# IIT-PAVIS/DiffAssemble

Measured on AMD Instinct MI355X. Metric: denoising steps/sec (900-piece dense graph, T=100), higher is better.
Workload: dtype bf16

## Files before the change

diffassemble_amd/csrc/da_basic.hip:

```cpp
#include "da_common.h"
#include "da_internal.h"

namespace da {

template <typename T>
__global__ __launch_bounds__(256) void k_set_feats(int n, int F, int D, const float *__restrict__ feats,
                                                   T *__restrict__ comb_in) {
    size_t total = (size_t)n * F;
    for (size_t idx = (size_t)blockIdx.x * blockDim.x + threadIdx.x; idx < total;
         idx += (size_t)gridDim.x * blockDim.x) {
        size_t r = idx / F;
        int c = (int)(idx - r * F);
        stf(comb_in + r * D + c, feats[idx]);
    }
}

template <typename T>
__global__ __launch_bounds__(256) void k_set_virtual_rows(int rows, int V, int D, const T *__restrict__ emb,
                                                          T *__restrict__ dst) {
    size_t total = (size_t)rows * D;
    for (size_t idx = (size_t)blockIdx.x * blockDim.x + threadIdx.x; idx < total;
         idx += (size_t)gridDim.x * blockDim.x) {
        size_t r = idx / D;
        int c = (int)(idx - r * D);
        dst[idx] = emb[(size_t)(r % V) * D + c];
    }
}

template <typename T>
__global__ __launch_bounds__(256) void k_embed_pos_time(int n, int NPW, int c_in, int F, int D, const float *__restrict__ x,
                                                        const int64_t *__restrict__ t, int64_t t_scalar, int steps,
                                                        const float *__restrict__ time_emb,
                                                        const float *__restrict__ w0, const float *__restrict__ b0,
                                                        const float *__restrict__ w1, const float *__restrict__ b1,
                                                        T *__restrict__ comb_in, int embed_blocks, VirtScatter vs) {
    __shared__ float hid[4][16];
    if ((int)blockIdx.x >= embed_blocks) {
        const int HC = vs.H * vs.C;
        const size_t total = (size_t)vs.rows * 4 * HC, stride = (size_t)(gridDim.x - embed_blocks) * blockDim.x;
        for (size_t idx = (size_t)(blockIdx.x - embed_blocks) * blockDim.x + threadIdx.x; idx < total; idx += stride) {
            const size_t r = idx / (4 * (size_t)HC);
            const int col = (int)(idx - r * 4 * HC), which = col / HC, f = col - which * HC;
            const T v = ((const T *)vs.src)[(size_t)(r % vs.V) * 4 * HC + col];
            const size_t node = (size_t)vs.n_real + r;
            if (which == 3) { ((T *)vs.S)[node * HC + f] = v; continue; }
            const int h = f / vs.C, c = f - h * vs.C;
            T *dstb = (T *)(which == 0 ? vs.Q : (which == 1 ? vs.K : vs.Vt));
            dstb[((size_t)h * (size_t)vs.n_pad + (size_t)vs.row_map[node]) * vs.C + c] = v;
        }
        return;
    }
    const int lane = threadIdx.x & 63, wv = threadIdx.x >> 6;
    const int r0 = (blockIdx.x * 4 + wv) * NPW;
    if (r0 >= n) return;
    float w0r[8], w1r[16];
    float b0r = 0.f, b1r = 0.f;
    if (lane < 16) {
        b0r = b0[lane];
#pragma unroll
        for (int k = 0; k < 8; ++k) w0r[k] = k < c_in ? w0[lane * c_in + k] : 0.f;
    }
    if (lane < 32) {
        b1r = b1[lane];
#pragma unroll
        for (int k = 0; k < 16; ++k) w1r[k] = w1[lane * 16 + k];
    }
    for (int i = 0; i < NPW; ++i) {
        const int r = r0 + i;
        if (r >= n) break;
        if (lane < 16) {
            float a = b0r;
#pragma unroll
            for (int k = 0; k < 8; ++k) a += k < c_in ? w0r[k] * x[(size_t)r * c_in + k] : 0.f;
            hid[wv][lane] = gelu_erf(a);
        }
        __builtin_amdgcn_wave_barrier();
        asm volatile("s_waitcnt lgkmcnt(0)" ::: "memory");
        T *dst = comb_in + (size_t)r * D + F;
        if (lane < 32) {
            float a = b1r;
#pragma unroll
            for (int k = 0; k < 16; ++k) a += w1r[k] * hid[wv][k];
            stf(dst + lane, a);
        } else {
            int64_t ti = t ? t[r] : t_scalar;
            ti = ti < 0 ? 0 : (ti >= steps ? steps - 1 : ti);
            stf(dst + lane, time_emb[ti * 32 + (lane - 32)]);
        }
        __builtin_amdgcn_wave_barrier();
    }
}

template <typename T>
__global__ __launch_bounds__(256) void k_gemm_simple(int M, int K, int Nout, const T *__restrict__ A, int lda,
                                                     const T *__restrict__ W, const float *__restrict__ bias,
                                                     int act, const T *__restrict__ res, T *__restrict__ out,
                                                     int ldo) {
    __shared__ float As[16][68];
    __shared__ float Ws[16][68];
    const int tx = threadIdx.x & 15, ty = threadIdx.x >> 4;
    const int row0 = blockIdx.y * 64, col0 = blockIdx.x * 64;
    const int lr = threadIdx.x >> 2, lk = (threadIdx.x & 3) * 4;
    float acc[4][4];
#pragma unroll
    for (int i = 0; i < 4; ++i)
#pragma unroll
        for (int j = 0; j < 4; ++j) acc[i][j] = 0.f;
    const int ar = row0 + lr, wr = col0 + lr;
    for (int k0 = 0; k0 < K; k0 += 16) {
#pragma unroll
        for (int i = 0; i < 4; ++i) {
            const int k = k0 + lk + i;
            As[lk + i][lr] = (ar < M && k < K) ? ldf(A + (size_t)ar * lda + k) : 0.f;
            Ws[lk + i][lr] = (wr < Nout && k < K) ? ldf(W + (size_t)wr * K + k) : 0.f;
        }
        __syncthreads();
#pragma unroll
        for (int kk = 0; kk < 16; ++kk) {
            float a[4], b[4];
#pragma unroll
            for (int i = 0; i < 4; ++i) { a[i] = As[kk][ty * 4 + i]; b[i] = Ws[kk][tx * 4 + i]; }
#pragma unroll
            for (int i = 0; i < 4; ++i)
#pragma unroll
                for (int j = 0; j < 4; ++j) acc[i][j] = fmaf(a[i], b[j], acc[i][j]);
        }
        __syncthreads();
    }
#pragma unroll
    for (int i = 0; i < 4; ++i) {
        const int r = row0 + ty * 4 + i;
        if (r >= M) continue;
#pragma unroll
        for (int j = 0; j < 4; ++j) {
            const int c = col0 + tx * 4 + j;
            if (c >= Nout) continue;
            float v = acc[i][j] + (bias ? bias[c] : 0.f);
            v = apply_act(v, act);
            if (res) v += ldf(res + (size_t)r * ldo + c);
            stf(out + (size_t)r * ldo + c, v);
        }
    }
}

template <typename T>
__global__ __launch_bounds__(256) void k_head2d(int n, int c_out, const T *__restrict__ hh,
                                                const float *__restrict__ w2, const float *__restrict__ b2,
                                                float *__restrict__ out) {
    const int idx = blockIdx.x * blockDim.x + threadIdx.x;
    if (idx >= n * c_out) return;
    const int r = idx / c_out, c = idx - r * c_out;
    float a = b2[c];
#pragma unroll
    for (int k = 0; k < 32; ++k) a += w2[c * 32 + k] * ldf(hh + (size_t)r * 32 + k);
    out[idx] = a;
}

__global__ __launch_bounds__(256) void k_ddim2d(DeviceSchedule s, int mean_type, int n, int c,
                                                const float *__restrict__ x, const float *__restrict__ mo,
                                                const int64_t *__restrict__ t, int64_t t_scalar, int ratio,
                                                int prev_all_nonneg, float eta, const float *__restrict__ noise,
                                                float *__restrict__ x_prev) {
    const int idx = blockIdx.x * blockDim.x + threadIdx.x;
    if (idx >= n * c) return;
    const int r = idx / c;
    const int64_t ti = t ? t[r] : t_scalar;
    x_prev[idx] = ddim2d_value(s, mean_type, ti, ratio, prev_all_nonneg, eta, x[idx], mo[idx], (eta > 0.f && noise) ? noise[idx] : 0.f);
}

__global__ __launch_bounds__(256) void k_ddpm2d(DeviceSchedule s, int n, int c, const float *__restrict__ x,
                                                const float *__restrict__ mo, const int64_t *__restrict__ t,
                                                int64_t t_scalar, const float *__restrict__ noise,
                                                float *__restrict__ x_prev) {
    const int idx = blockIdx.x * blockDim.x + threadIdx.x;
    if (idx >= n * c) return;
    const int r = idx / c;
    int64_t ti = t ? t[r] : t_scalar;
    ti = ti < 0 ? 0 : (ti >= s.steps ? s.steps - 1 : ti);
    float mean = s.sqrt_recip_alphas[ti] * (x[idx] - s.betas[ti] * mo[idx] / s.sqrt_one_minus_alphas_cumprod[ti]);
    if (noise) mean += sqrtf(s.posterior_variance[ti]) * noise[idx];
    x_prev[idx] = mean;
}

template <typename T>
__global__ __launch_bounds__(256) void k_convert(size_t n, const float *__restrict__ src, T *__restrict__ dst) {
    for (size_t i = (size_t)blockIdx.x * blockDim.x + threadIdx.x; i < n; i += (size_t)gridDim.x * blockDim.x)
        stf(dst + i, src[i]);
}

static inline int grid_for(size_t total, int block = 256, int cap = 4096) {
    size_t g = (total + block - 1) / block;
    return (int)(g < 1 ? 1 : (g > (size_t)cap ? cap : g));
}

template <typename T>
static int launch_set_feats_t(int n, int F, int D, const float *feats, void *comb_in, hipStream_t st) {
    if (n <= 0) return 0;
    k_set_feats<T><<<grid_for((size_t)n * F), 256, 0, st>>>(n, F, D, feats, (T *)comb_in);
    DA_LAUNCH_CHECK();
    return 0;
}
int launch_set_feats(int prec, int n, int F, int D, const float *feats, void *comb_in, hipStream_t st) {
    return prec == DA_PREC_BF16 ? launch_set_feats_t<bf16_t>(n, F, D, feats, comb_in, st)
                                : launch_set_feats_t<float>(n, F, D, feats, comb_in, st);
}

int launch_set_virtual_rows(int prec, int rows, int V, int D, const void *emb, void *dst, hipStream_t st) {
    if (rows <= 0) return 0;
    if (prec == DA_PREC_BF16)
        k_set_virtual_rows<bf16_t><<<grid_for((size_t)rows * D), 256, 0, st>>>(rows, V, D, (const bf16_t *)emb, (bf16_t *)dst);
    else
        k_set_virtual_rows<float><<<grid_for((size_t)rows * D), 256, 0, st>>>(rows, V, D, (const float *)emb, (float *)dst);
    DA_LAUNCH_CHECK();
    return 0;
}

int launch_embed_pos_time(int prec, int n, int c_in, int F, int D, const float *x, const int64_t *t, int64_t t_scalar,
                          int steps, const float *time_emb, const float *w0, const float *b0, const float *w1,
                          const float *b1, void *comb_in, hipStream_t st, const VirtScatter *vsp) {
    if (n <= 0) return 0;
    if (c_in > 8) { set_error("launch_embed_pos_time: c_in %d > 8", c_in); return 2; }
    VirtScatter vs;
    if (vsp && vsp->rows > 0) vs = *vsp;
    const size_t vtotal = (size_t)vs.rows * 4 * vs.H * vs.C;
    const int vblocks = vs.rows > 0 ? (int)((vtotal + 255) / 256 > 1024 ? 1024 : (vtotal + 255) / 256) : 0;
    const int npw_env = DA_XENV("DA_EMBED_NPW", 0);
    const int npw = npw_env > 0 ? npw_env : (n >= 8192 ? 8 : 1), grid = (n + 4 * npw - 1) / (4 * npw);
    if (prec == DA_PREC_BF16)
        k_embed_pos_time<bf16_t><<<grid + vblocks, 256, 0, st>>>(n, npw, c_in, F, D, x, t, t_scalar, steps, time_emb, w0, b0, w1, b1, (bf16_t *)comb_in, grid, vs);
    else
        k_embed_pos_time<float><<<grid + vblocks, 256, 0, st>>>(n, npw, c_in, F, D, x, t, t_scalar, steps, time_emb, w0, b0, w1, b1, (float *)comb_in, grid, vs);
    DA_LAUNCH_CHECK();
    return 0;
}

int launch_gemm_simple(int prec, int M, int K, int Nout, const void *A, int lda, const void *W, const float *bias,
                       int act, const void *res, void *out, int ldo, hipStream_t st) {
    if (M <= 0 || Nout <= 0) return 0;
    dim3 grid((Nout + 63) / 64, (M + 63) / 64);
    if (prec == DA_PREC_BF16)
        k_gemm_simple<bf16_t><<<grid, 256, 0, st>>>(M, K, Nout, (const bf16_t *)A, lda, (const bf16_t *)W, bias, act, (const bf16_t *)res, (bf16_t *)out, ldo);
    else
        k_gemm_simple<float><<<grid, 256, 0, st>>>(M, K, Nout, (const float *)A, lda, (const float *)W, bias, act, (const float *)res, (float *)out, ldo);
    DA_LAUNCH_CHECK();
    return 0;
}

int launch_head2d(int prec, int n, int c_out, const void *hh, const float *w2, const float *b2, float *out, hipStream_t st) {
    if (n <= 0) return 0;
    const int grid = (n * c_out + 255) / 256;
    if (prec == DA_PREC_BF16)
        k_head2d<bf16_t><<<grid, 256, 0, st>>>(n, c_out, (const bf16_t *)hh, w2, b2, out);
    else
        k_head2d<float><<<grid, 256, 0, st>>>(n, c_out, (const float *)hh, w2, b2, out);
    DA_LAUNCH_CHECK();
    return 0;
}

int launch_ddim2d(const DeviceSchedule &s, int mean_type, int n, int c, const float *x, const float *mo,
                  const int64_t *t, int64_t t_scalar, int ratio, int prev_all_nonneg, float eta, const float *noise,
                  float *x_prev, hipStream_t st) {
    if (n <= 0) return 0;
    k_ddim2d<<<(n * c + 255) / 256, 256, 0, st>>>(s, mean_type, n, c, x, mo, t, t_scalar, ratio, prev_all_nonneg, eta, noise, x_prev);
    DA_LAUNCH_CHECK();
    return 0;
}

int launch_ddpm2d(const DeviceSchedule &s, int n, int c, const float *x, const float *mo, const int64_t *t,
                  int64_t t_scalar, const float *noise, float *x_prev, hipStream_t st) {
    if (n <= 0) return 0;
    k_ddpm2d<<<(n * c + 255) / 256, 256, 0, st>>>(s, n, c, x, mo, t, t_scalar, noise, x_prev);
    DA_LAUNCH_CHECK();
    return 0;
}

int launch_convert(int prec, size_t n, const float *src, void *dst, hipStream_t st) {
    if (n == 0) return 0;
    if (prec == DA_PREC_BF16)
        k_convert<bf16_t><<<grid_for(n), 256, 0, st>>>(n, src, (bf16_t *)dst);
    else
        k_convert<float><<<grid_for(n), 256, 0, st>>>(n, src, (float *)dst);
    DA_LAUNCH_CHECK();
    return 0;
}


__global__ __launch_bounds__(256) void k_mm_nn_f32(int M, int N, int K, const float *__restrict__ A, int lda,
                                                   const float *__restrict__ B, int ldb, const float *__restrict__ bias,
                                                   float *__restrict__ Cm, int ldc) {
    const int idx = blockIdx.x * blockDim.x + threadIdx.x;
    if (idx >= M * N) return;
    const int m = idx / N, n = idx - m * N;
    float acc = 0.f;
    for (int k = 0; k < K; ++k) acc = fmaf(A[(size_t)m * lda + k], B[(size_t)k * ldb + n], acc);
    Cm[(size_t)m * ldc + n] = acc + (bias ? bias[m] : 0.f);
}

int launch_mm_nn_f32(int M, int N, int K, const float *A, int lda, const float *B, int ldb, const float *bias, float *Cm,
                     int ldc, hipStream_t st) {
    k_mm_nn_f32<<<(M * N + 255) / 256, 256, 0, st>>>(M, N, K, A, lda, B, ldb, bias, Cm, ldc);
    DA_LAUNCH_CHECK();
    return 0;
}

__device__ __forceinline__ void ld4f(const float *p, float (&v)[4]) {
    const float4 f = *(const float4 *)p;
    v[0] = f.x; v[1] = f.y; v[2] = f.z; v[3] = f.w;
}
__device__ __forceinline__ void ld4f(const bf16_t *p, float (&v)[4]) {
    const uint2 u = *(const uint2 *)p;
    v[0] = bf2f((bf16_t)(u.x & 0xffff)); v[1] = bf2f((bf16_t)(u.x >> 16));
    v[2] = bf2f((bf16_t)(u.y & 0xffff)); v[3] = bf2f((bf16_t)(u.y >> 16));
}
template <typename T>
__global__ __launch_bounds__(256) void k_head_fold(int n, int H, int c_out, const T *__restrict__ pz, const T *__restrict__ pre,
                                                   const float *__restrict__ w2, const float *__restrict__ b2,
                                                   float *__restrict__ out, DdimFuse df) {
    __shared__ float f[32][33];
    const int q = threadIdx.x & 7, lr = threadIdx.x >> 3;
    const int r = blockIdx.x * 32 + lr;
    if (r < n) {
        float a[4], v[4];
        ld4f(pre + (size_t)r * 32 + 4 * q, a);
        for (int h = 0; h < H; ++h) {
            ld4f(pz + ((size_t)h * n + r) * 32 + 4 * q, v);
#pragma unroll
            for (int e = 0; e < 4; ++e) a[e] += v[e];
        }
#pragma unroll
        for (int e = 0; e < 4; ++e) f[lr][4 * q + e] = gelu_erf(a[e]);
    }
    __syncthreads();
    const int lr2 = threadIdx.x / c_out, j = threadIdx.x - lr2 * c_out;
    const int r2 = blockIdx.x * 32 + lr2;
    if (lr2 < 32 && r2 < n) {
        float a = b2[j];
#pragma unroll
        for (int k = 0; k < 32; ++k) a = fmaf(w2[j * 32 + k], f[lr2][k], a);
        out[(size_t)r2 * c_out + j] = a;
        if (df.x_prev)
            df.x_prev[(size_t)r2 * c_out + j] = ddim2d_value(df.s, df.mean_type, df.t, df.ratio, df.prev_all_nonneg, 0.f,
                                                             df.x[(size_t)r2 * c_out + j], a, 0.f);
    }
}

typedef __attribute__((ext_vector_type(8))) __bf16 tl_bf16x8;
typedef __attribute__((ext_vector_type(16))) float tl_f32x16;
typedef __attribute__((ext_vector_type(4))) unsigned int tl_u32x4;
typedef __attribute__((ext_vector_type(4))) float f32x4_t;
template <bool NEXT>
__global__ __launch_bounds__(64) void k_tail_fused(int n, int H, int c_out, const bf16_t *h, const bf16_t *__restrict__ xin,
                                                   int ldx, const bf16_t *__restrict__ wh, const float *__restrict__ bh,
                                                   const bf16_t *__restrict__ wsk, const float *__restrict__ bsk,
                                                   const bf16_t *__restrict__ pz, const float *__restrict__ w2,
                                                   const float *__restrict__ b2, float *__restrict__ out, DdimFuse df, int slabs_per_wave) {
    constexpr int KH = 128, KX = 256, NCH = (KH + KX) / 16;
    const int lane = threadIdx.x, m = lane & 31, g = lane >> 5;
    tl_u32x4 wf[NCH];
#pragma unroll
    for (int c = 0; c < KH / 16; ++c) wf[c] = *(const tl_u32x4 *)(wh + (size_t)m * KH + 16 * c + 8 * g);
#pragma unroll
    for (int c = 0; c < KX / 16; ++c) wf[KH / 16 + c] = *(const tl_u32x4 *)(wsk + (size_t)m * KX + 16 * c + 8 * g);
    float bias[16];
#pragma unroll
    for (int r = 0; r < 16; ++r) { const int ch = (r & 3) + 8 * (r >> 2) + 4 * g; bias[r] = bh[ch] + bsk[ch]; }
    for (int sl = 0; sl < slabs_per_wave; ++sl) {
        const int row0 = (blockIdx.x * slabs_per_wave + sl) * 32;
        if (row0 >= n) break;
        const int row = min(row0 + m, n - 1);
        tl_u32x4 xf[NCH];
#pragma unroll
        for (int c = 0; c < KH / 16; ++c) xf[c] = *(const tl_u32x4 *)(h + (size_t)row * KH + 16 * c + 8 * g);
#pragma unroll
        for (int c = 0; c < KX / 16; ++c) xf[KH / 16 + c] = *(const tl_u32x4 *)(xin + (size_t)row * ldx + 16 * c + 8 * g);
        uint2 pzv[8][4];
#pragma unroll
        for (int hh = 0; hh < 8; ++hh)
#pragma unroll
            for (int q = 0; q < 4; ++q)
                pzv[hh][q] = hh < H ? *(const uint2 *)(pz + ((size_t)hh * n + row) * 32 + 8 * q + 4 * g) : make_uint2(0u, 0u);
        tl_f32x16 acc;
#pragma unroll
        for (int r = 0; r < 16; ++r) acc[r] = bias[r];
#pragma unroll
        for (int c = 0; c < NCH; ++c)
            acc = __builtin_amdgcn_mfma_f32_32x32x16_bf16(__builtin_bit_cast(tl_bf16x8, wf[c]), __builtin_bit_cast(tl_bf16x8, xf[c]), acc, 0, 0, 0);
        float f[16];
#pragma unroll
        for (int q = 0; q < 4; ++q) {
            float a[4] = {acc[4 * q], acc[4 * q + 1], acc[4 * q + 2], acc[4 * q + 3]};
#pragma unroll
            for (int hh = 0; hh < 8; ++hh) {
                const uint2 u = pzv[hh][q];
                a[0] += bf2f((bf16_t)(u.x & 0xffff)); a[1] += bf2f((bf16_t)(u.x >> 16));
                a[2] += bf2f((bf16_t)(u.y & 0xffff)); a[3] += bf2f((bf16_t)(u.y >> 16));
            }
#pragma unroll
            for (int e = 0; e < 4; ++e) f[4 * q + e] = gelu_erf(a[e]);
        }
        float xn[8] = {0.f, 0.f, 0.f, 0.f, 0.f, 0.f, 0.f, 0.f};
#pragma unroll
        for (int j = 0; j < 8; ++j) {
            if (j >= c_out) break;
            float part = 0.f;
#pragma unroll
            for (int r = 0; r < 16; ++r) {
                const int k0 = (r & 3) + 8 * (r >> 2);
                const float wlo = w2[j * 32 + k0], whi = w2[j * 32 + k0 + 4];
                part = fmaf(g ? whi : wlo, f[r], part);
            }
            const float a = b2[j] + part + __shfl_xor(part, 32);
            const size_t o = (size_t)row * c_out + j;
            if (df.x_prev) xn[j] = ddim2d_value(df.s, df.mean_type, df.t, df.ratio, df.prev_all_nonneg, 0.f, df.x[o], a, 0.f);
            if (g == 0 && row0 + m < n) {
                out[o] = a;
                if (df.x_prev) df.x_prev[o] = xn[j];
            }
        }
        if (NEXT) {
            const int cin = df.nx_cin;
            float hm[8];
#pragma unroll
            for (int kk = 0; kk < 8; ++kk) {
                float a = g ? df.nx_b0[8 + kk] : df.nx_b0[kk];
#pragma unroll
                for (int j = 0; j < 8; ++j)
                    if (j < cin) a += (g ? df.nx_w0[(8 + kk) * cin + j] : df.nx_w0[kk * cin + j]) * xn[j];
                hm[kk] = gelu_erf(a);
            }
            float hid[16];
#pragma unroll
            for (int kk = 0; kk < 8; ++kk) {
                const float ho = __shfl_xor(hm[kk], 32);
                hid[kk] = g ? ho : hm[kk];
                hid[8 + kk] = g ? hm[kk] : ho;
            }
            long long ti = df.nx_t;
            ti = ti < 0 ? 0 : (ti >= df.nx_steps ? df.nx_steps - 1 : ti);
            tl_u32x4 bx[4];
#pragma unroll
            for (int c = 0; c < 2; ++c) {
                unsigned pk[4];
#pragma unroll
                for (int e2 = 0; e2 < 4; ++e2) {
                    unsigned short two[2];
#pragma unroll
                    for (int z = 0; z < 2; ++z) {
                        const int o = 16 * c + 8 * g + 2 * e2 + z;
                        const f32x4_t *wr = (const f32x4_t *)(df.nx_w1 + (size_t)o * 16);
                        float a = df.nx_b1[o];
#pragma unroll
                        for (int q4 = 0; q4 < 4; ++q4) {
                            const f32x4_t w4 = wr[q4];
                            a += w4[0] * hid[4 * q4]; a += w4[1] * hid[4 * q4 + 1]; a += w4[2] * hid[4 * q4 + 2]; a += w4[3] * hid[4 * q4 + 3];
                        }
                        two[z] = f2bf(a);
                    }
                    pk[e2] = (unsigned)two[0] | ((unsigned)two[1] << 16);
                }
                bx[c] = (tl_u32x4){pk[0], pk[1], pk[2], pk[3]};
            }
#pragma unroll
            for (int c = 0; c < 2; ++c) {
                const f32x4_t *tr = (const f32x4_t *)(df.nx_time_emb + (size_t)ti * 32 + 16 * c + 8 * g);
                const f32x4_t t0 = tr[0], t1 = tr[1];
                bx[2 + c] = (tl_u32x4){(unsigned)f2bf(t0[0]) | ((unsigned)f2bf(t0[1]) << 16), (unsigned)f2bf(t0[2]) | ((unsigned)f2bf(t0[3]) << 16),
                                       (unsigned)f2bf(t1[0]) | ((unsigned)f2bf(t1[1]) << 16), (unsigned)f2bf(t1[2]) | ((unsigned)f2bf(t1[3]) << 16)};
            }
            const bf16_t *wp = (const bf16_t *)df.nx_wp;
            const bf16_t *fp = (const bf16_t *)df.nx_feat_proj + (size_t)row * 128;
            bf16_t *hn = (bf16_t *)df.nx_h + (size_t)row * 128;
#pragma unroll
            for (int mt = 0; mt < 4; ++mt) {
                tl_u32x4 wa[4];
#pragma unroll
                for (int c = 0; c < 4; ++c) wa[c] = *(const tl_u32x4 *)(wp + (size_t)(32 * mt + m) * df.nx_ldw + 16 * c + 8 * g);
                uint2 fpv[4];
#pragma unroll
                for (int q = 0; q < 4; ++q) fpv[q] = *(const uint2 *)(fp + 32 * mt + 8 * q + 4 * g);
                tl_f32x16 ac;
#pragma unroll
                for (int r = 0; r < 16; ++r) ac[r] = 0.f;
#pragma unroll
                for (int c = 0; c < 4; ++c)
                    ac = __builtin_amdgcn_mfma_f32_32x32x16_bf16(__builtin_bit_cast(tl_bf16x8, wa[c]), __builtin_bit_cast(tl_bf16x8, bx[c]), ac, 0, 0, 0);
#pragma unroll
                for (int q = 0; q < 4; ++q) {
                    float v[4] = {ac[4 * q] + bf2f((bf16_t)(fpv[q].x & 0xffff)), ac[4 * q + 1] + bf2f((bf16_t)(fpv[q].x >> 16)),
                                  ac[4 * q + 2] + bf2f((bf16_t)(fpv[q].y & 0xffff)), ac[4 * q + 3] + bf2f((bf16_t)(fpv[q].y >> 16))};
#pragma unroll
                    for (int e = 0; e < 4; ++e) v[e] = gelu_erf(v[e]);
                    if (row0 + m < n)
                        *(uint2 *)(hn + 32 * mt + 8 * q + 4 * g) = make_uint2((unsigned)f2bf(v[0]) | ((unsigned)f2bf(v[1]) << 16),
                                                                              (unsigned)f2bf(v[2]) | ((unsigned)f2bf(v[3]) << 16));
                }
            }
        }
    }
}

int launch_tail_fused(int prec, int n, int H, int c_out, int hidden, int din, const void *h, const void *xin, int ldx, const void *wh,
                      const float *bh, const void *wsk, const float *bsk, const void *pz, const float *w2, const float *b2, float *out,
                      hipStream_t st, DdimFuse *dfp) {
    const bool off = (cfg().disable_folds & DA_FOLD_TAIL) != 0;
    if (off || prec != DA_PREC_BF16 || hidden != 128 || din != 256 || H > 8 || c_out > 8 || (ldx & 7)) return -1;
    if (n <= 0) return 0;
    DdimFuse df;
    if (dfp) df = *dfp; else { df = DdimFuse(); df.x = nullptr; df.x_prev = nullptr; }
    const int slabs = (n + 31) / 32;
    int spw = (slabs + 1023) / 1024;
    spw = spw < 1 ? 1 : (spw > 4 ? 4 : spw);
    const bool nx_off = cfg().tail_next == 0;
    const bool next = dfp && df.x_prev && df.nx_on && !nx_off && df.nx_cin <= 8 && df.nx_cin == c_out && df.nx_h == h;
    if (next)
        k_tail_fused<true><<<(slabs + spw - 1) / spw, 64, 0, st>>>(n, H, c_out, (const bf16_t *)h, (const bf16_t *)xin, ldx, (const bf16_t *)wh, bh,
                                                                   (const bf16_t *)wsk, bsk, (const bf16_t *)pz, w2, b2, out, df, spw);
    else
        k_tail_fused<false><<<(slabs + spw - 1) / spw, 64, 0, st>>>(n, H, c_out, (const bf16_t *)h, (const bf16_t *)xin, ldx, (const bf16_t *)wh, bh,
                                                                    (const bf16_t *)wsk, bsk, (const bf16_t *)pz, w2, b2, out, df, spw);
    DA_LAUNCH_CHECK();
    if (next) dfp->nx_done = 1;
    return 0;
}

int launch_head_fold(int prec, int n, int H, int c_out, const void *pz, const void *pre, const float *w2, const float *b2,
                     float *out, hipStream_t st, const DdimFuse *dfp) {
    if (n <= 0) return 0;
    DdimFuse df;
    if (dfp) df = *dfp; else { df = DdimFuse(); df.x = nullptr; df.x_prev = nullptr; }
    if (c_out > 8) { set_error("launch_head_fold: c_out %d > 8", c_out); return 2; }
    if (prec == DA_PREC_BF16) k_head_fold<bf16_t><<<(n + 31) / 32, 256, 0, st>>>(n, H, c_out, (const bf16_t *)pz, (const bf16_t *)pre, w2, b2, out, df);
    else k_head_fold<float><<<(n + 31) / 32, 256, 0, st>>>(n, H, c_out, (const float *)pz, (const float *)pre, w2, b2, out, df);
    DA_LAUNCH_CHECK();
    return 0;
}


template <typename T>
__global__ __launch_bounds__(256) void k_scatter_virtual(int rows, int V, int H, int C, const T *__restrict__ src, int n_real,
                                                         const int32_t *__restrict__ row_map, size_t n_pad, T *Q, T *K, T *Vt,
                                                         T *S, T *qkvs) {
    const int HC = H * C;
    const size_t total = (size_t)rows * 4 * HC;
    for (size_t idx = (size_t)blockIdx.x * blockDim.x + threadIdx.x; idx < total; idx += (size_t)gridDim.x * blockDim.x) {
        const size_t r = idx / (4 * (size_t)HC);
        const int col = (int)(idx - r * 4 * HC), which = col / HC, f = col - which * HC;
        const T v = src[(size_t)(r % V) * 4 * HC + col];
        const size_t node = (size_t)n_real + r;
        if (qkvs) { qkvs[node * 4 * HC + col] = v; continue; }
        if (which == 3) { S[node * HC + f] = v; continue; }
        const int h = f / C, c = f - h * C;
        T *dstb = which == 0 ? Q : (which == 1 ? K : Vt);
        dstb[((size_t)h * n_pad + (size_t)row_map[node]) * C + c] = v;
    }
}

int launch_scatter_virtual(int prec, int rows, int V, int H, int C, const void *src, int n_real, const int32_t *row_map,
                           int n_pad, void *Q, void *K, void *Vt, void *S, void *qkvs, hipStream_t st) {
    if (rows <= 0) return 0;
    const size_t total = (size_t)rows * 4 * H * C;
    const unsigned grid = (unsigned)((total + 255) / 256 > 4096 ? 4096 : (total + 255) / 256);
    if (prec == DA_PREC_BF16)
        k_scatter_virtual<bf16_t><<<grid, 256, 0, st>>>(rows, V, H, C, (const bf16_t *)src, n_real, row_map, (size_t)n_pad,
                                                        (bf16_t *)Q, (bf16_t *)K, (bf16_t *)Vt, (bf16_t *)S, (bf16_t *)qkvs);
    else
        k_scatter_virtual<float><<<grid, 256, 0, st>>>(rows, V, H, C, (const float *)src, n_real, row_map, (size_t)n_pad,
                                                       (float *)Q, (float *)K, (float *)Vt, (float *)S, (float *)qkvs);
    DA_LAUNCH_CHECK();
    return 0;
}

}
```

diffassemble_amd/csrc/da_internal.h:

```cpp
#pragma once
#include "da_common.h"
#include "da_config.h"

namespace da {

struct DeviceSchedule {
    int steps;
    const float *betas, *alphas_cumprod, *sqrt_recip_alphas, *sqrt_recip_alphas_cumprod,
        *sqrt_recipm1_alphas_cumprod, *sqrt_one_minus_alphas_cumprod, *posterior_variance;
};
inline DeviceSchedule to_dev(const da_schedule *s) {
    return {s->steps, s->betas, s->alphas_cumprod, s->sqrt_recip_alphas, s->sqrt_recip_alphas_cumprod, s->sqrt_recipm1_alphas_cumprod,
            s->sqrt_one_minus_alphas_cumprod, s->posterior_variance};
}

__device__ __forceinline__ float ddim2d_value(const DeviceSchedule &s, int mean_type, long long ti, int ratio,
                                              int prev_all_nonneg, float eta, float xv, float m, float noise) {
    ti = ti < 0 ? 0 : (ti >= s.steps ? s.steps - 1 : ti);
    const long long tp = ti - ratio;
    const float ap = s.alphas_cumprod[ti];
    const float ap_prev = (prev_all_nonneg && tp >= 0) ? s.alphas_cumprod[tp] : 1.0f;
    const float beta = 1.0f - ap;
    const float x0 = mean_type == DA_MEAN_START_X ? m : (xv - sqrtf(beta) * m) / sqrtf(ap);
    const float eps = (s.sqrt_recip_alphas_cumprod[ti] * xv - x0) / s.sqrt_recipm1_alphas_cumprod[ti];
    const float var = ((1.0f - ap_prev) / (1.0f - ap)) * (1.0f - ap / ap_prev);
    const float std_eta = eta * sqrtf(var);
    float prev = sqrtf(ap_prev) * x0 + sqrtf(1.0f - ap_prev - std_eta * std_eta) * eps;
    if (eta > 0.f) prev += std_eta * noise;
    return prev;
}

struct DdimFuse {
    DeviceSchedule s;
    int mean_type, ratio, prev_all_nonneg;
    long long t;
    const float *x;
    float *x_prev;
    int done;
    int nx_on, nx_done, nx_steps, nx_cin, nx_ldw;
    long long nx_t;
    const float *nx_time_emb, *nx_w0, *nx_b0, *nx_w1, *nx_b1;
    const void *nx_wp;
    const void *nx_feat_proj;
    void *nx_h;
};

int launch_set_feats(int prec, int n, int F, int D, const float *feats, void *comb_in, hipStream_t st);
int launch_set_virtual_rows(int prec, int rows, int V, int D, const void *emb, void *dst, hipStream_t st);
struct VirtScatter {
    int rows = 0, V = 0, H = 0, C = 0, n_real = 0, n_pad = 0;
    const void *src = nullptr;
    const int32_t *row_map = nullptr;
    void *Q = nullptr, *K = nullptr, *Vt = nullptr, *S = nullptr;
};
int launch_embed_pos_time(int prec, int n, int c_in, int F, int D, const float *x, const int64_t *t, int64_t t_scalar,
                          int steps, const float *time_emb, const float *w0, const float *b0, const float *w1,
                          const float *b1, void *comb_in, hipStream_t st, const VirtScatter *vs = nullptr);
int launch_gemm_simple(int prec, int M, int K, int Nout, const void *A, int lda, const void *W, const float *bias,
                       int act, const void *res, void *out, int ldo, hipStream_t st);
int launch_head2d(int prec, int n, int c_out, const void *hh, const float *w2, const float *b2, float *out, hipStream_t st);
int launch_ddim2d(const DeviceSchedule &s, int mean_type, int n, int c, const float *x, const float *mo,
                  const int64_t *t, int64_t t_scalar, int ratio, int prev_all_nonneg, float eta, const float *noise,
                  float *x_prev, hipStream_t st);
int launch_ddpm2d(const DeviceSchedule &s, int n, int c, const float *x, const float *mo, const int64_t *t,
                  int64_t t_scalar, const float *noise, float *x_prev, hipStream_t st);
int launch_convert(int prec, size_t n, const float *src, void *dst, hipStream_t st);
int launch_transpose_f32(int rows, int cols, const float *src, float *dst, hipStream_t st);
int launch_gemm_tn(int M, int N, int K, const float *A, int lda, const float *B, int ldb, float *C, int ldc, float *partial,
                   hipStream_t st, bool bfc = false);
int launch_gemm_tn_bf16(int M, int N, int K, const bf16_t *A, int lda, const bf16_t *B, int ldb, float *C, int ldc, float *partial,
                        hipStream_t st);
int launch_gemm_mfma_splitk(int M, int K, int Nout, const void *A, int lda, const void *W, const float *bias, const void *res,
                            void *out, int ldo, float *partial, size_t partial_floats, hipStream_t st, bool in16 = false,
                            const float *gelu_pre = nullptr, float *act_out = nullptr);
int launch_gemm_mfma_mixed(bool in16, bool out16, int M, int K, int Nout, const void *A, int lda, const void *W, const float *bias,
                           const void *res, void *out, int ldo, hipStream_t st);
int launch_gemm_tn_db(int M, int N, int K, const void *A, int lda, const void *B, int ldb, float *C, int ldc, float *partial,
                      float *db, float *bscratch, hipStream_t st, bool a16 = false, bool b16 = false);
int colsum_add(int M, int N, const float *A, int lda, float *out, float *scratch, hipStream_t st);
int launch_conv(int prec, int B, const void *X, int Cin, int Hi, const void *W, const float *bias, const void *res, void *Y,
                int Cout, int ksize, int stride, int relu, hipStream_t st);
int launch_enc_stem(int prec, int B, const float *patches, const float *w, const float *bias, void *Y, int relu, hipStream_t st);
int launch_mm_nn_f32(int M, int N, int K, const float *A, int lda, const float *B, int ldb, const float *bias, float *C,
                     int ldc, hipStream_t st);
int launch_scatter_virtual(int prec, int rows, int V, int H, int C, const void *src, int n_real, const int32_t *row_map,
                           int n_pad, void *Q, void *K, void *Vt, void *S, void *qkvs, hipStream_t st);
int launch_tail_fused(int prec, int n, int H, int c_out, int hidden, int din, const void *h, const void *xin, int ldx, const void *wh,
                      const float *bh, const void *wsk, const float *bsk, const void *pz, const float *w2, const float *b2, float *out,
                      hipStream_t st, DdimFuse *dfp);
int launch_head_fold(int prec, int n, int H, int c_out, const void *pz, const void *pre, const float *w2, const float *b2,
                     float *out, hipStream_t st, const DdimFuse *df = nullptr);

int launch_attn_tiny(int prec, int n_graphs, int max_graph_nodes, const int32_t *graph_ptr, int nodiag, int heads, int C, const void *qkvs,
                     const void *residual, int act, void *out, hipStream_t st);
int launch_attn_csr(int prec, int n_nodes, const int32_t *row_ptr, const int32_t *col_src, const int32_t *edge_id,
                    int heads, int C, const void *qkvs, const void *residual, int act, void *out, float *alpha,
                    float *stats , hipStream_t st);

int launch_head3d(int prec, int n, const void *hh, const float *wt, const float *bt, const float *wr, const float *br,
                  float *out7, float *pre_head, hipStream_t st);
int launch_head3d_bwd(int n, const float *pre, const float *d_out, float *d_pre, hipStream_t st);
int launch_ddim3d(const DeviceSchedule &s, int mean_type, int n, const float *x, const float *mo, const int64_t *t,
                  int64_t t_scalar, int ratio, int prev_all_nonneg, float *x_prev, hipStream_t st);

struct StreamJoin {
    hipStream_t side = nullptr, caller = nullptr;
    hipEvent_t ev = nullptr;
    bool armed = false;
    void arm(hipStream_t side_, hipStream_t caller_, hipEvent_t ev_) { side = side_; caller = caller_; ev = ev_; armed = true; }
    hipError_t join() {
        if (!armed) return hipSuccess;
        armed = false;
        hipError_t e = hipEventRecord(ev, side);
        return e == hipSuccess ? hipStreamWaitEvent(caller, ev, 0) : e;
    }
    ~StreamJoin() { (void)join(); }
};
struct QkvScatter {
    int HC, C, n_pad;
    int Cv = 0;
    int blocks = 0;
    int col0 = 0;
    const int32_t *row_map;
    void *Q, *K, *Vt, *S;
};
struct DenseLayout {
    const void *Q, *K, *Vt, *S;
    int n_pad;
    int q_prescaled = 0;
    const void *x = nullptr;
    int ldx = 0, kin = 0;
    const void *wqs = nullptr;
    const float *bias = nullptr;
    bool x_fm = false, out_fm = false;
};
bool attn_qsf_applicable(int prec, int heads, int C, int kin, int n_graphs, int max_graph_nodes, int n_pad, int q_prescaled);
bool attn_qsf_enabled();
bool attn_last_qproj_applicable(int prec, int heads, int C, int kin, int n_pad, int q_prescaled);
bool attn_last_qproj_enabled();
size_t w_qlast_bytes(int heads, int C, int kin);
int pack_w_qlast(int heads, int C, int kin, const void *wq, void *packed, hipStream_t st);
long long attn_last_qproj_launches(int reset);
size_t w_qs_bytes(int heads, int kin);
int pack_w_qs(int heads, int kin, int hc, const void *wd, void *packed, hipStream_t st);
int launch_gemm_mfma(int prec, int M, int K, int Nout, const void *A, int lda, const void *W, const float *bias,
                     int act, const void *res, void *out, int ldo, const QkvScatter *qs, hipStream_t st, int ldw = 0,
                     const void *pre = nullptr, const void *wpacked = nullptr);
size_t xpanel_packed_bytes(int K, int Nout);
bool xpanel_in_model();
void gemm_thin_set(int v);
int xpanel_mode();
int pack_w_xpanel(int K, int Nout, const void *W, int ldw, void *packed, hipStream_t st);
struct DenseMask {
    const uint8_t *mask;
    const int64_t *mask_ptr;
    const int32_t *irr_row_ptr, *irr_col_src, *row_map;
    const int32_t *slot_node = nullptr;
    const uint8_t *blk_class = nullptr;
    const int64_t *blk_class_ptr = nullptr;
    int blk_class_stride = 0;
    const int32_t *rm_meta = nullptr;
    int v_rows = 0, v_n_real = 0;
    const int32_t *v_row_ptr = nullptr, *v_col_src = nullptr;
    const float *v_mult = nullptr;
    float *v_part = nullptr;
    unsigned *v_cnt = nullptr;
    int *v_taken = nullptr;
};
constexpr int DA_VIRT_SPLIT_MAX = 8;
inline DenseMask dense_mask_of(const da_graph *g) {
    DenseMask mk;
    mk.mask = g->mask; mk.mask_ptr = g->mask_ptr; mk.irr_row_ptr = g->irr_row_ptr; mk.irr_col_src = g->irr_col_src; mk.row_map = g->row_map;
    mk.slot_node = g->slot_node;
    mk.rm_meta = g->rm_meta;
    const bool cls = g->blk_class && g->blk_class_ptr && g->blk_class_stride > 0;
    mk.blk_class = cls ? g->blk_class : nullptr; mk.blk_class_ptr = cls ? g->blk_class_ptr : nullptr; mk.blk_class_stride = cls ? g->blk_class_stride : 0;
    return mk;
}
struct DenseFold {
    int cv;
    void *out;
    int n_rows;
};
int launch_attn_dense(int prec, const DenseLayout &L, int heads, int C, int n_graphs, int max_graph_nodes,
                      const int32_t *graph_ptr, const int32_t *pad_ptr, int nodiag, const void *res, int act,
                      void *out, hipStream_t st, const DenseMask *mk = nullptr, const DenseFold *fold = nullptr);
int launch_attn_dual(const DenseLayout &L, int heads, int C, int n_graphs, int max_graph_nodes, const int32_t *graph_ptr,
                     const int32_t *pad_ptr, int nodiag, int act, void *out, const DenseFold *fold, hipStream_t st);
int attn_dense_counters(unsigned long long *out4, int reset);
long long attn_virt_launches(int reset);
long long attn_res_launches(int reset);
long long attn_res_qsf_launches(int reset);
long long attn_res_fm_launches(int reset);
int attn_dual_counters(unsigned long long *out2, int reset);
int launch_attn_csr_cont(int prec, int n_nodes, int n_real, const int32_t *irr_row_ptr, const int32_t *irr_col_src,
                         const int32_t *row_map, int heads, int C, int n_pad, const DenseLayout &L,
                         const void *residual, int act, void *out, hipStream_t st,
                         const float *mult = nullptr );

bool conv_fused_applicable(int prec, int heads, int C, int kin, int max_graph_nodes, int ldo);
int launch_conv_fused(int prec, int heads, int C, int kin, int n_graphs, int max_graph_nodes, const int32_t *graph_ptr,
                      int nodiag, const void *x, int ldx, const void *W, const float *bias, int act, void *out, int ldo,
                      hipStream_t st);

int pcd_knn_launch(int clouds, int N, int dim, const float *x, int ldx, int32_t *idx, const float *xn, hipStream_t st);
int pcd_premap_launch(int C, const float *X, int ldx, const float *Wm, long long total, float *T, hipStream_t st);
int pcd_edge_launch(const float *T, const int32_t *idx, const float *bn_a, const float *wb, int N, int clouds, float *Xout,
                    float *xn, hipStream_t st);
int pcd_conv6_final_launch(const float *X1, const float *X2, const float *X3, const float *w6, int feat, int N, int clouds,
                           float *partial, const float *lin0, int inv, float *out, int ldo, hipStream_t st);

int gcn_plan_kind(const da_graph *g);
int launch_gcn_dinv(const da_graph *g, float *dinv, hipStream_t st);
int launch_gcn_aggregate(int prec, const da_graph *g, int W, const float *dinv, const void *X, const float *bias, int act, void *out,
                         hipStream_t st);
int launch_gcn_aggregate_t(int prec, const da_graph *g, int W, const float *dinv, const void *X, void *out, hipStream_t st);
int launch_gcn_gelu_res(size_t n, const float *pre, const float *res, float *out, hipStream_t st);

struct D3pmStep {
    DeviceSchedule s = {};
    const int32_t *x_t = nullptr;
    const int64_t *t = nullptr;
    int64_t t_scalar = 0;
    int ratio = 1;
    const float *noise = nullptr;
    const uint64_t *seed = nullptr;
    int iteration = 0;
    int32_t *x_prev = nullptr;
    float *post = nullptr;
};
int launch_embed_idx_time(int prec, int n, int K, int F, int D, const int32_t *idx, const int64_t *t, int64_t t_scalar, int steps,
                          const float *time_emb, const float *pos_emb, void *comb_in, hipStream_t st);
struct D3pmRows {
    const void *hh = nullptr, *pz = nullptr, *pre = nullptr;
};
constexpr uint32_t D3PM_WORD_SAMPLING = 0xD3B07384u, D3PM_WORD_TRAINING = 0x51ED270Bu;
constexpr uint32_t D3PM_WORD_SAMPLING_ROT = 0x2A65C0F1u;
constexpr uint32_t D3PM_WORD_TRAINING_ROT = 0x7C3A91E5u;
inline uint32_t d3pm_domain_word(int domain) {
    return domain == DA_D3PM_DRAW_TRAINING ? D3PM_WORD_TRAINING : domain == DA_D3PM_DRAW_SAMPLING_ROT ? D3PM_WORD_SAMPLING_ROT :
           domain == DA_D3PM_DRAW_TRAINING_ROT ? D3PM_WORD_TRAINING_ROT : D3PM_WORD_SAMPLING;
}
__device__ __forceinline__ float philox_uniform(uint64_t seed, uint64_t ctr, uint32_t iteration, uint32_t word = D3PM_WORD_SAMPLING) {
    uint32_t c0 = (uint32_t)ctr, c1 = (uint32_t)(ctr >> 32), c2 = iteration, c3 = word;
    uint32_t k0 = (uint32_t)seed, k1 = (uint32_t)(seed >> 32);
#pragma unroll
    for (int i = 0; i < 10; ++i) {
        const uint32_t hi0 = __umulhi(0xD2511F53u, c0), lo0 = 0xD2511F53u * c0;
        const uint32_t hi1 = __umulhi(0xCD9E8D57u, c2), lo1 = 0xCD9E8D57u * c2;
        c0 = hi1 ^ c1 ^ k0; c1 = lo1; c2 = hi0 ^ c3 ^ k1; c3 = lo0;
        k0 += 0x9E3779B9u; k1 += 0xBB67AE85u;
    }
    return (float)((c0 >> 8) + 1u) * 5.9604644775390625e-8f;
}
int launch_embed_idx_grad(int n, int K, int D, int F, const int32_t *idx, const float *dcomb, float *grad, hipStream_t st);
int launch_d3pm_q_sample(int n, int K, const da_schedule *s, const int32_t *x_start, const int32_t *rot_start, const int64_t *t,
                         const float *noise_x, const float *noise_rot, const uint64_t *seed, int iteration, int32_t *x_noisy,
                         int32_t *rot_noisy, hipStream_t st);
int launch_d3pm_tail(int prec, int n, int K, int H, const D3pmRows *rows_c, const D3pmRows *rows_u, float cfg_w, const float *w2,
                     const float *b2, const float *logits_in, float *logits_out, const D3pmStep *step, hipStream_t st);

int launch_embed_idx_time_rot(int prec, int n, int K, int F, int D, int hidden, const int32_t *idx, const int32_t *rot_acc, const int64_t *t,
                              int64_t t_scalar, int steps, const float *time_emb, const float *pos_emb, void *comb_in, const void *proj4,
                              size_t img_stride, void *sel, hipStream_t st);
struct D3pmRotStep {
    DeviceSchedule s = {};
    const int32_t *x_t = nullptr, *rot_t = nullptr;
    const int64_t *t = nullptr;
    int64_t t_scalar = 0;
    int ratio = 1;
    const float *noise_x = nullptr, *noise_rot = nullptr;
    const uint64_t *seed = nullptr;
    int iteration = 0;
    int32_t *x_prev = nullptr, *rot_0 = nullptr, *rot_prev = nullptr;
    float *post_x = nullptr, *post_rot = nullptr;
    int cold = 0, need_prev = 1;
    const int32_t *rot_acc_in = nullptr;
    int32_t *rot_next = nullptr, *rot_acc_out = nullptr;
};
int launch_d3pm_rot_tail(int prec, int n, int K, const void *hh, const float *w2, const float *b2, const float *wr, const float *br,
                         const float *logits_in, const float *rot_logits_in, float *logits_out, float *rot_logits_out,
                         const D3pmRotStep *step, hipStream_t st);

int linear(int prec, int M, int K, int Nout, const void *A, int lda, const void *W, const float *bias, int act,
           const void *res, void *out, int ldo, hipStream_t st);

}
```

Baseline: 109,200.

## Stage tail-fused kernel constants in LDS via async global_load_lds and specialize on c_out

```diff
diff --git a/diffassemble_amd/csrc/da_basic.hip b/diffassemble_amd/csrc/da_basic.hip
--- a/diffassemble_amd/csrc/da_basic.hip
+++ b/diffassemble_amd/csrc/da_basic.hip
@@ -348,26 +348,58 @@
 typedef __attribute__((ext_vector_type(16))) float tl_f32x16;
 typedef __attribute__((ext_vector_type(4))) unsigned int tl_u32x4;
 typedef __attribute__((ext_vector_type(4))) float f32x4_t;
-template <bool NEXT>
+constexpr int TL_W2 = 0, TL_B2 = 256, TL_BH = 320, TL_BS = 352, TL_W0 = 384, TL_B0 = 512, TL_B1 = 576, TL_TE = 608, TL_W1 = 640, TL_WP = 1152, TL_FP = 5248,
+              TL_END = 7296;
+typedef __attribute__((address_space(1))) const void tl_glb_t;
+typedef __attribute__((address_space(3))) void tl_lds_t;
+#define TL_GLDS(gp, lp, bytes) __builtin_amdgcn_global_load_lds((tl_glb_t *)(gp), (tl_lds_t *)(lp), bytes, 0, 0)
+template <bool NEXT, int C>
 __global__ __launch_bounds__(64) void k_tail_fused(int n, int H, int c_out, const bf16_t *h, const bf16_t *__restrict__ xin,
                                                    int ldx, const bf16_t *__restrict__ wh, const float *__restrict__ bh,
                                                    const bf16_t *__restrict__ wsk, const float *__restrict__ bsk,
                                                    const bf16_t *__restrict__ pz, const float *__restrict__ w2,
                                                    const float *__restrict__ b2, float *__restrict__ out, DdimFuse df, int slabs_per_wave) {
     constexpr int KH = 128, KX = 256, NCH = (KH + KX) / 16;
+    constexpr int NW2 = C ? (C * 32 + 63) / 64 : 4, NW0 = C ? (C * 16 + 63) / 64 : 2;
+    __shared__ __attribute__((aligned(16))) float tab[NEXT ? TL_END : TL_W0];
     const int lane = threadIdx.x, m = lane & 31, g = lane >> 5;
+    const int cc = C ? C : c_out;
+    const bool ddim = df.x_prev != nullptr;
+#pragma unroll
+    for (int k = 0; k < NW2; ++k) TL_GLDS(w2 + min(lane + 64 * k, cc * 32 - 1), tab + TL_W2 + 64 * k, 4);
+    TL_GLDS(b2 + min(lane, cc - 1), tab + TL_B2, 4);
+    TL_GLDS(lane < 32 ? bh + lane : bsk + (lane - 32), tab + TL_BH, 4);
+    if (NEXT) {
+        long long ti = df.nx_t;
+        ti = ti < 0 ? 0 : (ti >= df.nx_steps ? df.nx_steps - 1 : ti);
+#pragma unroll
+        for (int k = 0; k < NW0; ++k) TL_GLDS(df.nx_w0 + min(lane + 64 * k, cc * 16 - 1), tab + TL_W0 + 64 * k, 4);
+        TL_GLDS(df.nx_b0 + (lane & 15), tab + TL_B0, 4);
+        TL_GLDS(lane < 32 ? df.nx_b1 + lane : df.nx_time_emb + (size_t)ti * 32 + (lane - 32), tab + TL_B1, 4);
+#pragma unroll
+        for (int k = 0; k < 2; ++k) TL_GLDS(df.nx_w1 + 4 * (lane + 64 * k), tab + TL_W1 + 256 * k, 16);
+        const bf16_t *wp = (const bf16_t *)df.nx_wp;
+#pragma unroll
+        for (int mt = 0; mt < 4; ++mt)
+#pragma unroll
+            for (int c = 0; c < 4; ++c) TL_GLDS(wp + (size_t)(32 * mt + m) * df.nx_ldw + 16 * c + 8 * g, tab + TL_WP + 256 * (4 * mt + c), 16);
+    }
+    DdimCoeffs kf = {1.f, 1.f, 1.f, 1.f, true};
+    if (ddim) kf = ddim2d_coeffs(df.s, df.t, df.ratio, df.prev_all_nonneg);
     tl_u32x4 wf[NCH];
 #pragma unroll
     for (int c = 0; c < KH / 16; ++c) wf[c] = *(const tl_u32x4 *)(wh + (size_t)m * KH + 16 * c + 8 * g);
 #pragma unroll
     for (int c = 0; c < KX / 16; ++c) wf[KH / 16 + c] = *(const tl_u32x4 *)(wsk + (size_t)m * KX + 16 * c + 8 * g);
-    float bias[16];
-#pragma unroll
-    for (int r = 0; r < 16; ++r) { const int ch = (r & 3) + 8 * (r >> 2) + 4 * g; bias[r] = bh[ch] + bsk[ch]; }
     for (int sl = 0; sl < slabs_per_wave; ++sl) {
         const int row0 = (blockIdx.x * slabs_per_wave + sl) * 32;
         if (row0 >= n) break;
         const int row = min(row0 + m, n - 1);
+        if (NEXT) {
+            const bf16_t *fp = (const bf16_t *)df.nx_feat_proj + (size_t)row * 128;
+#pragma unroll
+            for (int k = 0; k < 8; ++k) TL_GLDS(fp + 16 * k + 8 * g, tab + TL_FP + 256 * k, 16);
+        }
         tl_u32x4 xf[NCH];
 #pragma unroll
         for (int c = 0; c < KH / 16; ++c) xf[c] = *(const tl_u32x4 *)(h + (size_t)row * KH + 16 * c + 8 * g);
@@ -379,9 +411,22 @@
 #pragma unroll
             for (int q = 0; q < 4; ++q)
                 pzv[hh][q] = hh < H ? *(const uint2 *)(pz + ((size_t)hh * n + row) * 32 + 8 * q + 4 * g) : make_uint2(0u, 0u);
+        float xr[C ? C : 8];
+        if (ddim) {
+            if (C == 4) { const float4 v = *(const float4 *)(df.x + (size_t)row * 4); xr[0] = v.x; xr[1] = v.y; xr[2] = v.z; xr[3] = v.w; }
+            else if (C == 2) { const float2 v = *(const float2 *)(df.x + (size_t)row * 2); xr[0] = v.x; xr[1] = v.y; }
+            else {
+#pragma unroll
+                for (int j = 0; j < 8; ++j) xr[j] = df.x[(size_t)row * cc + min(j, cc - 1)];
+            }
+        } else {
+#pragma unroll
+            for (int j = 0; j < (C ? C : 8); ++j) xr[j] = 0.f;
+        }
+        asm volatile("s_waitcnt vmcnt(0)" : "+v"(kf.ap), "+v"(kf.ap_tp), "+v"(kf.recip), "+v"(kf.recipm1) : : "memory");
         tl_f32x16 acc;
 #pragma unroll
-        for (int r = 0; r < 16; ++r) acc[r] = bias[r];
+        for (int r = 0; r < 16; ++r) { const int ch = (r & 3) + 8 * (r >> 2) + 4 * g; acc[r] = tab[TL_BH + ch] + tab[TL_BS + ch]; }
 #pragma unroll
         for (int c = 0; c < NCH; ++c)
             acc = __builtin_amdgcn_mfma_f32_32x32x16_bf16(__builtin_bit_cast(tl_bf16x8, wf[c]), __builtin_bit_cast(tl_bf16x8, xf[c]), acc, 0, 0, 0);
@@ -398,34 +443,44 @@
 #pragma unroll
             for (int e = 0; e < 4; ++e) f[4 * q + e] = gelu_erf(a[e]);
         }
-        float xn[8] = {0.f, 0.f, 0.f, 0.f, 0.f, 0.f, 0.f, 0.f};
-#pragma unroll
-        for (int j = 0; j < 8; ++j) {
-            if (j >= c_out) break;
+        float xn[C ? C : 8], av[C ? C : 8];
+#pragma unroll
+        for (int j = 0; j < (C ? C : 8); ++j) { xn[j] = 0.f; av[j] = 0.f; }
+#pragma unroll
+        for (int j = 0; j < (C ? C : 8); ++j) {
+            if (!C && j >= c_out) break;
             float part = 0.f;
 #pragma unroll
             for (int r = 0; r < 16; ++r) {
                 const int k0 = (r & 3) + 8 * (r >> 2);
-                const float wlo = w2[j * 32 + k0], whi = w2[j * 32 + k0 + 4];
-                part = fmaf(g ? whi : wlo, f[r], part);
-            }
-            const float a = b2[j] + part + __shfl_xor(part, 32);
-            const size_t o = (size_t)row * c_out + j;
-            if (df.x_prev) xn[j] = ddim2d_value(df.s, df.mean_type, df.t, df.ratio, df.prev_all_nonneg, 0.f, df.x[o], a, 0.f);
-            if (g == 0 && row0 + m < n) {
+                part = fmaf(tab[TL_W2 + j * 32 + k0 + 4 * g], f[r], part);
+            }
+            const float a = tab[TL_B2 + j] + part + __shfl_xor(part, 32);
+            av[j] = a;
+            if (ddim) xn[j] = ddim2d_apply(kf, df.mean_type, 0.f, xr[j], a, 0.f);
+            if (!C && g == 0 && row0 + m < n) {
+                const size_t o = (size_t)row * c_out + j;
                 out[o] = a;
-                if (df.x_prev) df.x_prev[o] = xn[j];
-            }
+                if (ddim) df.x_prev[o] = xn[j];
+            }
+        }
+        if (C == 4 && g == 0 && row0 + m < n) {
+            *(float4 *)(out + (size_t)row * 4) = make_float4(av[0], av[1], av[2], av[3]);
+            if (ddim) *(float4 *)(df.x_prev + (size_t)row * 4) = make_float4(xn[0], xn[1], xn[2], xn[3]);
+        }
+        if (C == 2 && g == 0 && row0 + m < n) {
+            *(float2 *)(out + (size_t)row * 2) = make_float2(av[0], av[1]);
+            if (ddim) *(float2 *)(df.x_prev + (size_t)row * 2) = make_float2(xn[0], xn[1]);
         }
         if (NEXT) {
-            const int cin = df.nx_cin;
+            const int cin = cc;
             float hm[8];
 #pragma unroll
             for (int kk = 0; kk < 8; ++kk) {
-                float a = g ? df.nx_b0[8 + kk] : df.nx_b0[kk];
-#pragma unroll
-                for (int j = 0; j < 8; ++j)
-                    if (j < cin) a += (g ? df.nx_w0[(8 + kk) * cin + j] : df.nx_w0[kk * cin + j]) * xn[j];
+                float a = tab[TL_B0 + 8 * g + kk];
+#pragma unroll
+                for (int j = 0; j < (C ? C : 8); ++j)
+                    if (j < cin) a = fmaf(tab[TL_W0 + (8 * g + kk) * cin + j], xn[j], a);
                 hm[kk] = gelu_erf(a);
             }
             float hid[16];
@@ -435,8 +490,6 @@
                 hid[kk] = g ? ho : hm[kk];
                 hid[8 + kk] = g ? hm[kk] : ho;
             }
-            long long ti = df.nx_t;
-            ti = ti < 0 ? 0 : (ti >= df.nx_steps ? df.nx_steps - 1 : ti);
             tl_u32x4 bx[4];
 #pragma unroll
             for (int c = 0; c < 2; ++c) {
@@ -447,8 +500,8 @@
 #pragma unroll
                     for (int z = 0; z < 2; ++z) {
                         const int o = 16 * c + 8 * g + 2 * e2 + z;
-                        const f32x4_t *wr = (const f32x4_t *)(df.nx_w1 + (size_t)o * 16);
-                        float a = df.nx_b1[o];
+                        const f32x4_t *wr = (const f32x4_t *)(tab + TL_W1 + o * 16);
+                        float a = tab[TL_B1 + o];
 #pragma unroll
                         for (int q4 = 0; q4 < 4; ++q4) {
                             const f32x4_t w4 = wr[q4];
@@ -462,32 +515,25 @@
             }
 #pragma unroll
             for (int c = 0; c < 2; ++c) {
-                const f32x4_t *tr = (const f32x4_t *)(df.nx_time_emb + (size_t)ti * 32 + 16 * c + 8 * g);
+                const f32x4_t *tr = (const f32x4_t *)(tab + TL_TE + 16 * c + 8 * g);
                 const f32x4_t t0 = tr[0], t1 = tr[1];
                 bx[2 + c] = (tl_u32x4){(unsigned)f2bf(t0[0]) | ((unsigned)f2bf(t0[1]) << 16), (unsigned)f2bf(t0[2]) | ((unsigned)f2bf(t0[3]) << 16),
                                        (unsigned)f2bf(t1[0]) | ((unsigned)f2bf(t1[1]) << 16), (unsigned)f2bf(t1[2]) | ((unsigned)f2bf(t1[3]) << 16)};
             }
-            const bf16_t *wp = (const bf16_t *)df.nx_wp;
-            const bf16_t *fp = (const bf16_t *)df.nx_feat_proj + (size_t)row * 128;
             bf16_t *hn = (bf16_t *)df.nx_h + (size_t)row * 128;
 #pragma unroll
             for (int mt = 0; mt < 4; ++mt) {
-                tl_u32x4 wa[4];
-#pragma unroll
-                for (int c = 0; c < 4; ++c) wa[c] = *(const tl_u32x4 *)(wp + (size_t)(32 * mt + m) * df.nx_ldw + 16 * c + 8 * g);
-                uint2 fpv[4];
-#pragma unroll
-                for (int q = 0; q < 4; ++q) fpv[q] = *(const uint2 *)(fp + 32 * mt + 8 * q + 4 * g);
                 tl_f32x16 ac;
 #pragma unroll
                 for (int r = 0; r < 16; ++r) ac[r] = 0.f;
 #pragma unroll
                 for (int c = 0; c < 4; ++c)
-                    ac = __builtin_amdgcn_mfma_f32_32x32x16_bf16(__builtin_bit_cast(tl_bf16x8, wa[c]), __builtin_bit_cast(tl_bf16x8, bx[c]), ac, 0, 0, 0);
+                    ac = __builtin_amdgcn_mfma_f32_32x32x16_bf16(__builtin_bit_cast(tl_bf16x8, *(const tl_u32x4 *)(tab + (NEXT ? TL_WP + 256 * (4 * mt + c) : 0) + 4 * lane)), __builtin_bit_cast(tl_bf16x8, bx[c]), ac, 0, 0, 0);
 #pragma unroll
                 for (int q = 0; q < 4; ++q) {
-                    float v[4] = {ac[4 * q] + bf2f((bf16_t)(fpv[q].x & 0xffff)), ac[4 * q + 1] + bf2f((bf16_t)(fpv[q].x >> 16)),
-                                  ac[4 * q + 2] + bf2f((bf16_t)(fpv[q].y & 0xffff)), ac[4 * q + 3] + bf2f((bf16_t)(fpv[q].y >> 16))};
+                    const uint2 fq = *(const uint2 *)(tab + (NEXT ? TL_FP + 256 * (2 * mt + (q >> 1)) : 0) + 4 * (32 * (q & 1) + m) + 2 * g);
+                    float v[4] = {ac[4 * q] + bf2f((bf16_t)(fq.x & 0xffff)), ac[4 * q + 1] + bf2f((bf16_t)(fq.x >> 16)),
+                                  ac[4 * q + 2] + bf2f((bf16_t)(fq.y & 0xffff)), ac[4 * q + 3] + bf2f((bf16_t)(fq.y >> 16))};
 #pragma unroll
                     for (int e = 0; e < 4; ++e) v[e] = gelu_erf(v[e]);
                     if (row0 + m < n)
@@ -512,12 +558,14 @@
     spw = spw < 1 ? 1 : (spw > 4 ? 4 : spw);
     const bool nx_off = cfg().tail_next == 0;
     const bool next = dfp && df.x_prev && df.nx_on && !nx_off && df.nx_cin <= 8 && df.nx_cin == c_out && df.nx_h == h;
-    if (next)
-        k_tail_fused<true><<<(slabs + spw - 1) / spw, 64, 0, st>>>(n, H, c_out, (const bf16_t *)h, (const bf16_t *)xin, ldx, (const bf16_t *)wh, bh,
-                                                                   (const bf16_t *)wsk, bsk, (const bf16_t *)pz, w2, b2, out, df, spw);
-    else
-        k_tail_fused<false><<<(slabs + spw - 1) / spw, 64, 0, st>>>(n, H, c_out, (const bf16_t *)h, (const bf16_t *)xin, ldx, (const bf16_t *)wh, bh,
-                                                                    (const bf16_t *)wsk, bsk, (const bf16_t *)pz, w2, b2, out, df, spw);
+    const uintptr_t rows_at = (uintptr_t)out | (uintptr_t)df.x | (uintptr_t)df.x_prev;
+    const int ci = (c_out == 4 && !(rows_at & 15)) ? 4 : (c_out == 2 && !(rows_at & 7)) ? 2 : 0;
+#define DA_TAIL_LAUNCH(NX, CI)                                                                                                                  \
+    k_tail_fused<NX, CI><<<(slabs + spw - 1) / spw, 64, 0, st>>>(n, H, c_out, (const bf16_t *)h, (const bf16_t *)xin, ldx, (const bf16_t *)wh, bh, \
+                                                                 (const bf16_t *)wsk, bsk, (const bf16_t *)pz, w2, b2, out, df, spw)
+    if (next) { if (ci == 4) DA_TAIL_LAUNCH(true, 4); else if (ci == 2) DA_TAIL_LAUNCH(true, 2); else DA_TAIL_LAUNCH(true, 0); }
+    else      { if (ci == 4) DA_TAIL_LAUNCH(false, 4); else if (ci == 2) DA_TAIL_LAUNCH(false, 2); else DA_TAIL_LAUNCH(false, 0); }
+#undef DA_TAIL_LAUNCH
     DA_LAUNCH_CHECK();
     if (next) dfp->nx_done = 1;
     return 0;
diff --git a/diffassemble_amd/csrc/da_internal.h b/diffassemble_amd/csrc/da_internal.h
--- a/diffassemble_amd/csrc/da_internal.h
+++ b/diffassemble_amd/csrc/da_internal.h
@@ -14,20 +14,32 @@
             s->sqrt_one_minus_alphas_cumprod, s->posterior_variance};
 }
 
-__device__ __forceinline__ float ddim2d_value(const DeviceSchedule &s, int mean_type, long long ti, int ratio,
-                                              int prev_all_nonneg, float eta, float xv, float m, float noise) {
+struct DdimCoeffs { float ap, ap_tp, recip, recipm1; bool prev_one; };
+__device__ __forceinline__ DdimCoeffs ddim2d_coeffs(const DeviceSchedule &s, long long ti, int ratio, int prev_all_nonneg) {
     ti = ti < 0 ? 0 : (ti >= s.steps ? s.steps - 1 : ti);
     const long long tp = ti - ratio;
-    const float ap = s.alphas_cumprod[ti];
-    const float ap_prev = (prev_all_nonneg && tp >= 0) ? s.alphas_cumprod[tp] : 1.0f;
+    DdimCoeffs k;
+    k.ap = s.alphas_cumprod[ti];
+    k.ap_tp = s.alphas_cumprod[tp >= 0 ? tp : 0];
+    k.prev_one = !(prev_all_nonneg && tp >= 0);
+    k.recip = s.sqrt_recip_alphas_cumprod[ti];
+    k.recipm1 = s.sqrt_recipm1_alphas_cumprod[ti];
+    return k;
+}
+__device__ __forceinline__ float ddim2d_apply(const DdimCoeffs &k, int mean_type, float eta, float xv, float m, float noise) {
+    const float ap = k.ap, ap_prev = k.prev_one ? 1.0f : k.ap_tp;
     const float beta = 1.0f - ap;
     const float x0 = mean_type == DA_MEAN_START_X ? m : (xv - sqrtf(beta) * m) / sqrtf(ap);
-    const float eps = (s.sqrt_recip_alphas_cumprod[ti] * xv - x0) / s.sqrt_recipm1_alphas_cumprod[ti];
+    const float eps = (k.recip * xv - x0) / k.recipm1;
     const float var = ((1.0f - ap_prev) / (1.0f - ap)) * (1.0f - ap / ap_prev);
     const float std_eta = eta * sqrtf(var);
     float prev = sqrtf(ap_prev) * x0 + sqrtf(1.0f - ap_prev - std_eta * std_eta) * eps;
     if (eta > 0.f) prev += std_eta * noise;
     return prev;
+}
+__device__ __forceinline__ float ddim2d_value(const DeviceSchedule &s, int mean_type, long long ti, int ratio,
+                                              int prev_all_nonneg, float eta, float xv, float m, float noise) {
+    return ddim2d_apply(ddim2d_coeffs(s, ti, ratio, prev_all_nonneg), mean_type, eta, xv, m, noise);
 }
 
 struct DdimFuse {
```

New measurement: 110,200 (median of 6 runs). Within noise of the previous version (+0.9%).
